# ZhangHaoyang493/News_Recsys

Hardware: AMD Instinct MI355X
Metric: impressions/sec at batch 65536 (embedding hot path forward) (higher is better)
Workload: dtype f32

## Files before the change

news_recsys_amd/csrc/nrx_interact.hip:

```cpp
#include "nrx_common.h"

namespace {

__global__ __launch_bounds__(NRX_BLOCK) void bag_pool_fwd_kernel(const float* __restrict__ emb, const float* __restrict__ mask,
                                                                 int64_t batch, int L, int D, float* __restrict__ out) {
    const int64_t total = batch * (int64_t)D;
    for (int64_t i = (int64_t)blockIdx.x * NRX_BLOCK + threadIdx.x; i < total; i += (int64_t)gridDim.x * NRX_BLOCK) {
        const int64_t b = i / D;
        const int d = (int)(i - b * D);
        const float* e = emb + (b * L) * (int64_t)D + d;
        float acc = 0.f, den = 0.f;
        if (mask != nullptr) {
            const float* m = mask + b * (int64_t)L;
            for (int l = 0; l < L; ++l) {
#pragma clang fp contract(off)
                const float w = m[l];
                den += w;
                acc += e[(int64_t)l * D] * w;
            }
            out[i] = acc / (den + 1e-8f);
        } else {
            for (int l = 0; l < L; ++l) acc += e[(int64_t)l * D];
            out[i] = acc / (float)L;
        }
    }
}

template <bool VEC>
__global__ __launch_bounds__(NRX_BLOCK) void bag_pool_bwd_kernel(const float* __restrict__ g_out, const float* __restrict__ mask,
                                                                 int64_t batch, int L, int D, float* __restrict__ g_emb) {
    const int lane = threadIdx.x & 63;
    const int64_t wave = (int64_t)blockIdx.x * (NRX_BLOCK / 64) + (threadIdx.x >> 6);
    const int64_t nwaves = (int64_t)gridDim.x * (NRX_BLOCK / 64);
    const int n = L * D;
    for (int64_t b = wave; b < batch; b += nwaves) {
        float den = (float)L;
        if (mask != nullptr) {
            float part = 0.f;
            for (int l = lane; l < L; l += NRX_WAVE) part += mask[b * (int64_t)L + l];
            den = nrx_wave_sum(part) + 1e-8f;
        }
        const float* gb = g_out + b * (int64_t)D;
        const float* mb = mask ? mask + b * (int64_t)L : nullptr;
        float* ob = g_emb + b * (int64_t)n;
        if (VEC) {
            const unsigned q = (unsigned)D >> 2;
            for (unsigned e4 = lane; e4 < (unsigned)n >> 2; e4 += NRX_WAVE) {
                const unsigned l = e4 / q, d = (e4 - l * q) * 4;
                const float4 g = *reinterpret_cast<const float4*>(gb + d);
                const float m = mb ? mb[l] : 1.0f;
                float4 o = make_float4(g.x / den, g.y / den, g.z / den, g.w / den);
                if (mb) o = make_float4(o.x * m, o.y * m, o.z * m, o.w * m);
                *reinterpret_cast<float4*>(ob + (size_t)e4 * 4) = o;
            }
        } else {
            for (int e = lane; e < n; e += NRX_WAVE) {
                const int l = e / D, d = e - l * D;
                const float g = gb[d] / den;
                ob[e] = mb ? g * mb[l] : g;
            }
        }
    }
}

__device__ __forceinline__ float4 ld4(const float* p, int k0, int D, bool vec) {
    float4 v;
    if (vec) {
        v = *reinterpret_cast<const float4*>(p);
    } else {
        v.x = p[0];
        v.y = (k0 + 1 < D) ? p[1] : 0.f;
        v.z = (k0 + 2 < D) ? p[2] : 0.f;
        v.w = (k0 + 3 < D) ? p[3] : 0.f;
    }
    return v;
}

template <int QLOG2>
__global__ __launch_bounds__(NRX_BLOCK) void fm_fwd_kernel(const float* __restrict__ feat, int64_t ld, int F, int D,
                                                           int64_t batch, float* __restrict__ fm_out, bool vec,
                                                           float* __restrict__ sums = nullptr, int64_t sums_ld = 0) {
    constexpr int Q = 1 << QLOG2;
    constexpr int TB = NRX_BLOCK / Q;
    const int q = threadIdx.x & (Q - 1);
    const int64_t b = (int64_t)blockIdx.x * TB + (threadIdx.x >> QLOG2);
    const bool live = b < batch;
    float total = 0.f;
    for (int kc = 0; kc < D; kc += 4 * Q) {
        const int k0 = kc + q * 4;
        float first = 0.f;
        float4 s = make_float4(0.f, 0.f, 0.f, 0.f), sq = s;
        if (live && k0 < D) {
            const float* row = feat + b * ld + k0;
            for (int f = 0; f < F; ++f) {
                float4 v = ld4(row + (int64_t)f * D, k0, D, vec);
                if (k0 == 0) { first += v.x; v.x = 0.f; }
                s.x += v.x; s.y += v.y; s.z += v.z; s.w += v.w;
                sq.x += v.x * v.x; sq.y += v.y * v.y; sq.z += v.z * v.z; sq.w += v.w * v.w;
            }
        }
        total += 0.5f * ((s.x * s.x - sq.x) + (s.y * s.y - sq.y) + (s.z * s.z - sq.z) + (s.w * s.w - sq.w)) + first;
        if (sums != nullptr && live && k0 < D) {
            float* dst = sums + b * sums_ld + k0;
            const float v0 = k0 == 0 ? first : s.x;
            dst[0] = v0;
            if (k0 + 1 < D) dst[1] = s.y;
            if (k0 + 2 < D) dst[2] = s.z;
            if (k0 + 3 < D) dst[3] = s.w;
        }
    }
#pragma unroll
    for (int off = Q / 2; off > 0; off >>= 1) total += __shfl_xor(total, off, 64);
    if (live && q == 0) fm_out[b] = total;
}

template <int QLOG2>
__global__ __launch_bounds__(NRX_BLOCK) void fm_bwd_kernel(const float* __restrict__ feat, int64_t ld, int F, int D, int64_t batch,
                                                           const float* __restrict__ g_fm, const float* g_in, int64_t g_in_ld,
                                                           float* g_feat, int64_t g_ld, bool vec) {
    constexpr int Q = 1 << QLOG2;
    constexpr int TB = NRX_BLOCK / Q;
    constexpr int U = 8;
    const int q = threadIdx.x & (Q - 1);
    const int64_t b = (int64_t)blockIdx.x * TB + (threadIdx.x >> QLOG2);
    if (b >= batch) return;
    const float gl = g_fm[b];
    const bool gvec = vec && (g_ld & 3) == 0 && ((reinterpret_cast<uintptr_t>(g_feat) & 15u) == 0) &&
                      (g_in == nullptr || ((g_in_ld & 3) == 0 && (reinterpret_cast<uintptr_t>(g_in) & 15u) == 0));
    for (int kc = 0; kc < D; kc += 4 * Q) {
        const int k0 = kc + q * 4;
        if (k0 >= D) continue;
        const float* row = feat + b * ld + k0;
        const float* irow = g_in ? g_in + b * g_in_ld + k0 : nullptr;
        float* grow = g_feat + b * g_ld + k0;
        float4 s = make_float4(0.f, 0.f, 0.f, 0.f);
        int f = 0;
        for (; f + U <= F; f += U) {
            float4 v[U];
#pragma unroll
            for (int u = 0; u < U; ++u) v[u] = ld4(row + (int64_t)(f + u) * D, k0, D, vec);
#pragma unroll
            for (int u = 0; u < U; ++u) { s.x += v[u].x; s.y += v[u].y; s.z += v[u].z; s.w += v[u].w; }
        }
        for (; f < F; ++f) {
            const float4 v = ld4(row + (int64_t)f * D, k0, D, vec);
            s.x += v.x; s.y += v.y; s.z += v.z; s.w += v.w;
        }
        f = 0;
        if (gvec && k0 + 4 <= D) {
            for (; f + U <= F; f += U) {
                float4 v[U], up[U];
#pragma unroll
                for (int u = 0; u < U; ++u) {
                    v[u] = ld4(row + (int64_t)(f + u) * D, k0, D, vec);
                    up[u] = irow ? *reinterpret_cast<const float4*>(irow + (int64_t)(f + u) * D) : make_float4(0.f, 0.f, 0.f, 0.f);
                }
#pragma unroll
                for (int u = 0; u < U; ++u) {
                    float4 g = make_float4(gl * (s.x - v[u].x), gl * (s.y - v[u].y), gl * (s.z - v[u].z), gl * (s.w - v[u].w));
                    if (k0 == 0) g.x = gl;
                    *reinterpret_cast<float4*>(grow + (int64_t)(f + u) * D) = make_float4(up[u].x + g.x, up[u].y + g.y, up[u].z + g.z, up[u].w + g.w);
                }
            }
        }
        for (; f < F; ++f) {
            const float4 v = ld4(row + (int64_t)f * D, k0, D, vec);
            float g[4] = {gl * (s.x - v.x), gl * (s.y - v.y), gl * (s.z - v.z), gl * (s.w - v.w)};
            if (k0 == 0) g[0] = gl;
            float* gp = grow + (int64_t)f * D;
            const float* ip = irow ? irow + (int64_t)f * D : nullptr;
#pragma unroll
            for (int j = 0; j < 4; ++j)
                if (k0 + j < D) gp[j] = (ip ? ip[j] : 0.f) + g[j];
        }
    }
}

template <int R, int V>
struct RowRegs {
    float v[R][V];
};

template <int R, int V>
__device__ __forceinline__ void row_load(RowRegs<R, V>& x, const float* p, int D, int lane) {
#pragma unroll
    for (int r = 0; r < R; ++r) {
        const int c = (r * 64 + lane) * V;
        if (V == 4) {
            float4 t = make_float4(0.f, 0.f, 0.f, 0.f);
            if (c < D) t = *reinterpret_cast<const float4*>(p + c);
            x.v[r][0] = t.x; x.v[r][1 % V] = t.y; x.v[r][2 % V] = t.z; x.v[r][3 % V] = t.w;
        } else {
            x.v[r][0] = (c < D) ? p[c] : 0.f;
        }
    }
}
// ... 526 lines not shown
            NRX_GLOBAL nrx_f32x4* o = (NRX_GLOBAL nrx_f32x4*)(a->out + b * a->out_ld);
#pragma unroll
            for (int u = EARLY ? N : 0; u < 2 * N; ++u) {
                const float4 v = u < N ? x0[u] : xl[u - N];
                nrx_f32x4 t;
                t.x = v.x; t.y = v.y; t.z = v.z; t.w = v.w;
                NRX_GLOBAL nrx_f32x4* dst = o + (u < N ? 0 : W / 4) + (u < N ? u : u - N) * Q + q;
                if (STNT) __builtin_nontemporal_store(t, dst);
                else *dst = t;
            }
        }
    }
}

int ceil_log2i(int x) {
    int l = 0;
    while ((1 << l) < x) ++l;
    return l;
}

unsigned stream_grid(int64_t items, int per_block) {
    int64_t g = (items + per_block - 1) / per_block;
    const int64_t cap = 256 * 8;
    if (g > cap) g = cap;
    if (g < 1) g = 1;
    return (unsigned)g;
}

#define NRX_QSWITCH(qlog2, ...)               \
    switch (qlog2) {                           \
        case 0: { constexpr int QL = 0; __VA_ARGS__; } break; \
        case 1: { constexpr int QL = 1; __VA_ARGS__; } break; \
        case 2: { constexpr int QL = 2; __VA_ARGS__; } break; \
        case 3: { constexpr int QL = 3; __VA_ARGS__; } break; \
        case 4: { constexpr int QL = 4; __VA_ARGS__; } break; \
        case 5: { constexpr int QL = 5; __VA_ARGS__; } break; \
        default: { constexpr int QL = 6; __VA_ARGS__; } break; \
    }

#define NRX_RSWITCH(R_, V_, ...)                                   \
    if (V_ == 4) {                                                  \
        constexpr int VV = 4;                                       \
        if (R_ <= 1) { constexpr int RR = 1; __VA_ARGS__; }                \
        else if (R_ <= 2) { constexpr int RR = 2; __VA_ARGS__; }           \
        else if (R_ <= 4) { constexpr int RR = 4; __VA_ARGS__; }           \
        else { constexpr int RR = 8; __VA_ARGS__; }                        \
    } else {                                                        \
        constexpr int VV = 1;                                       \
        if (R_ <= 1) { constexpr int RR = 1; __VA_ARGS__; }                \
        else if (R_ <= 2) { constexpr int RR = 2; __VA_ARGS__; }           \
        else if (R_ <= 4) { constexpr int RR = 4; __VA_ARGS__; }           \
        else if (R_ <= 8) { constexpr int RR = 8; __VA_ARGS__; }           \
        else if (R_ <= 16) { constexpr int RR = 16; __VA_ARGS__; }         \
        else { constexpr int RR = 32; __VA_ARGS__; }                       \
    }

}

extern "C" int nrx_bag_pool_fwd(const float* emb, const float* mask, int64_t batch, int32_t bag_len,
                                int32_t dim, float* out, void* stream) {
    NRX_TRACE();
    NRX_REQUIRE(emb && out && batch >= 0 && bag_len >= 1 && dim >= 1, "nrx_bag_pool_fwd: bad argument");
    if (batch == 0) return NRX_OK;
    hipLaunchKernelGGL(bag_pool_fwd_kernel, dim3(stream_grid(batch * dim, NRX_BLOCK)), dim3(NRX_BLOCK), 0,
                       reinterpret_cast<hipStream_t>(stream), emb, mask, batch, bag_len, dim, out);
    NRX_LAUNCH_CHECK("nrx_bag_pool_fwd");
    return NRX_OK;
}

extern "C" int nrx_bag_pool_bwd(const float* g_out, const float* mask, int64_t batch, int32_t bag_len,
                                int32_t dim, float* g_emb, void* stream) {
    NRX_TRACE();
    NRX_REQUIRE(g_out && g_emb && batch >= 0 && bag_len >= 1 && dim >= 1, "nrx_bag_pool_bwd: bad argument");
    if (batch == 0) return NRX_OK;
    const bool vec = (dim & 3) == 0 && nrx_aligned16(g_out) && nrx_aligned16(g_emb);
    if (vec) hipLaunchKernelGGL(bag_pool_bwd_kernel<true>, dim3(stream_grid(batch, NRX_BLOCK / 64)), dim3(NRX_BLOCK), 0,
                                reinterpret_cast<hipStream_t>(stream), g_out, mask, batch, bag_len, dim, g_emb);
    else hipLaunchKernelGGL(bag_pool_bwd_kernel<false>, dim3(stream_grid(batch, NRX_BLOCK / 64)), dim3(NRX_BLOCK), 0,
                            reinterpret_cast<hipStream_t>(stream), g_out, mask, batch, bag_len, dim, g_emb);
    NRX_LAUNCH_CHECK("nrx_bag_pool_bwd");
    return NRX_OK;
}

extern "C" int nrx_fm_fwd(const float* feat, int64_t ld, int32_t n_fields, int32_t dim, int64_t batch,
                          float* fm_out, void* stream) {
    NRX_TRACE();
    NRX_REQUIRE(feat && fm_out && n_fields >= 1 && dim >= 1 && batch >= 0 && ld >= (int64_t)n_fields * dim,
                "nrx_fm_fwd: bad argument");
    if (batch == 0) return NRX_OK;
    int ql = ceil_log2i((dim + 3) / 4);
    if (ql > 6) ql = 6;
    const bool vec = (dim & 3) == 0 && (ld & 3) == 0 && nrx_aligned16(feat);
    const int tb = NRX_BLOCK >> ql;
    const unsigned grid = (unsigned)((batch + tb - 1) / tb);
    NRX_QSWITCH(ql, { hipLaunchKernelGGL((fm_fwd_kernel<QL>), dim3(grid), dim3(NRX_BLOCK), 0, reinterpret_cast<hipStream_t>(stream),
                                         feat, ld, n_fields, dim, batch, fm_out, vec); });
    NRX_LAUNCH_CHECK("nrx_fm_fwd");
    return NRX_OK;
}

extern "C" int nrx_fm_fwd_train(const float* feat, int64_t ld, int32_t n_fields, int32_t dim, int64_t batch,
                                float* fm_out, float* fm_sums, int64_t sums_ld, void* stream) {
    NRX_TRACE();
    NRX_REQUIRE(feat && fm_out && fm_sums && n_fields >= 1 && dim >= 1 && batch >= 0 && ld >= (int64_t)n_fields * dim && sums_ld >= dim,
                "nrx_fm_fwd_train: bad argument");
    if (batch == 0) return NRX_OK;
    int ql = ceil_log2i((dim + 3) / 4);
    if (ql > 6) ql = 6;
    const bool vec = (dim & 3) == 0 && (ld & 3) == 0 && nrx_aligned16(feat);
    const int tb = NRX_BLOCK >> ql;
    const unsigned grid = (unsigned)((batch + tb - 1) / tb);
    NRX_QSWITCH(ql, { hipLaunchKernelGGL((fm_fwd_kernel<QL>), dim3(grid), dim3(NRX_BLOCK), 0, reinterpret_cast<hipStream_t>(stream),
                                         feat, ld, n_fields, dim, batch, fm_out, vec, fm_sums, sums_ld); });
    NRX_LAUNCH_CHECK("nrx_fm_fwd_train");
    return NRX_OK;
}

extern "C" int nrx_fm_bwd(const float* feat, int64_t ld, int32_t n_fields, int32_t dim, int64_t batch,
                          const float* g_fm, const float* g_in, int64_t g_in_ld, float* g_feat, int64_t g_ld, void* stream) {
    NRX_TRACE();
    NRX_REQUIRE(feat && g_fm && g_feat && n_fields >= 1 && dim >= 1 && batch >= 0, "nrx_fm_bwd: bad argument");
    if (batch == 0) return NRX_OK;
    int ql = ceil_log2i((dim + 3) / 4);
    if (ql > 6) ql = 6;
    const bool vec = (dim & 3) == 0 && (ld & 3) == 0 && nrx_aligned16(feat);
    const int tb = NRX_BLOCK >> ql;
    const unsigned grid = (unsigned)((batch + tb - 1) / tb);
    NRX_QSWITCH(ql, { hipLaunchKernelGGL((fm_bwd_kernel<QL>), dim3(grid), dim3(NRX_BLOCK), 0, reinterpret_cast<hipStream_t>(stream),
                                         feat, ld, n_fields, dim, batch, g_fm, g_in, g_in_ld, g_feat, g_ld, vec); });
    NRX_LAUNCH_CHECK("nrx_fm_bwd");
    return NRX_OK;
}

namespace {
constexpr int FH_BLOCKS = 64;
__global__ __launch_bounds__(NRX_BLOCK) void fm_head_fwd_kernel(const float* __restrict__ logit, const float* __restrict__ bias, float* __restrict__ out,
                                                                int64_t batch) {
    const float b = bias != nullptr ? bias[0] : 0.f;
    for (int64_t i = (int64_t)blockIdx.x * NRX_BLOCK + threadIdx.x; i < batch; i += (int64_t)gridDim.x * NRX_BLOCK) {
        const float x = b + logit[i];
        out[i] = 1.0f / (1.0f + expf(-x));
    }
}
__global__ __launch_bounds__(NRX_BLOCK) void fm_head_bwd_kernel(const float* __restrict__ g_out, int64_t g_stride, const float* __restrict__ out,
                                                                float* __restrict__ g_logit, float* __restrict__ g_bias, uint32_t* __restrict__ state,
                                                                int64_t batch) {
    __shared__ float s_w[NRX_BLOCK / 64];
    __shared__ uint32_t s_last;
    const int64_t chunk = (batch + gridDim.x - 1) / gridDim.x;
    const int64_t lo = (int64_t)blockIdx.x * chunk, hi = lo + chunk < batch ? lo + chunk : batch;
    float acc = 0.f;
    for (int64_t i = lo + threadIdx.x; i < hi; i += NRX_BLOCK) {
        const float p = out[i];
        const float g = g_out[i * g_stride] * (p * (1.0f - p));
        g_logit[i] = g;
        acc += g;
    }
    if (g_bias == nullptr) return;
    acc = nrx_wave_sum(acc);
    if ((threadIdx.x & 63) == 0) s_w[threadIdx.x >> 6] = acc;
    __syncthreads();
    float* partial = reinterpret_cast<float*>(state + 8);
    if (threadIdx.x == 0) {
        partial[blockIdx.x] = (s_w[0] + s_w[1]) + (s_w[2] + s_w[3]);
        __threadfence();
        s_last = atomicAdd(&state[0], 1u) == gridDim.x - 1 ? 1u : 0u;
    }
    __syncthreads();
    if (s_last && threadIdx.x < 64) {
        __threadfence();
        float v = (int)threadIdx.x < (int)gridDim.x ? __hip_atomic_load(&partial[threadIdx.x], __ATOMIC_RELAXED, __HIP_MEMORY_SCOPE_AGENT) : 0.f;
        v = nrx_wave_sum(v);
        if (threadIdx.x == 0) {
            g_bias[0] = v;
            state[0] = 0;
        }
    }
}
}

extern "C" int nrx_fm_head_fwd(const float* logit, const float* bias, float* out, int64_t batch, void* stream) {
    NRX_TRACE();
    NRX_REQUIRE(logit && out && batch >= 0, "nrx_fm_head_fwd: bad argument");
    if (batch == 0) return NRX_OK;
    const int64_t g = (batch + NRX_BLOCK - 1) / NRX_BLOCK;
    hipLaunchKernelGGL(fm_head_fwd_kernel, dim3((unsigned)(g < 1024 ? g : 1024)), dim3(NRX_BLOCK), 0, reinterpret_cast<hipStream_t>(stream), logit, bias, out, batch);
    NRX_LAUNCH_CHECK("nrx_fm_head_fwd");
    return NRX_OK;
}

extern "C" int64_t nrx_fm_head_state_bytes(void) { return 32 + FH_BLOCKS * 4; }

// ... 326 lines not shown
```

news_recsys_amd/csrc/nrx_route_feat.hip:

```cpp
#include <cstring>

#include "nrx_common.h"

namespace {

constexpr int RF_THREADS = 256;
#ifndef NRX_RF_ROUNDS
#define NRX_RF_ROUNDS 16
#endif
constexpr int RF_ROUNDS = NRX_RF_ROUNDS;
constexpr int RF_TILE = RF_THREADS * RF_ROUNDS;
constexpr int RF_WAVES = RF_THREADS / 64;
constexpr int RF_MAX_WORLD = 64;

struct RouteFeatArgs {
    const void* ids[NRX_MAX_FEATURES];
    int64_t batch;
    int64_t capf;
    int32_t n_feats, world, idx64, tiles;
    int32_t* send_ids;
    int32_t* send_pos;
    int32_t* slot;
    int64_t* counts;
    int64_t* overflow;
// ... 379 lines not shown
    if (last_of_feat) {
        tiles_before_in_group(a->tile0[f], s_feat);
        groups_before(a->tile0[f], s_feat);
    }
#endif
    __syncthreads();
    const int64_t cap = a->cap, B = a->batch;
    const int L = a->bag_len[f];
    const uint64_t magic_l = a->magic_len[f];
    const int32_t tag0 = (int32_t)(f * B);
    const int64_t ntag_r = (int64_t)n * B;
#pragma unroll
    for (int j = 0; j < RF_ROUNDS; ++j) {
        if (owner[j] < 0) continue;
        const int o = owner[j];
        const int64_t i = i0 + j * RF_THREADS + tid;
        const int pt = RUNS ? rank[j] : s_cell[j * RF_WAVES + wid][o] + rank[j];
        const int64_t k = (int64_t)s_base[o] + pt;
        const int32_t smp = RUNS ? (int32_t)smp0 + local_sample(j) : (L == 1 ? (int32_t)i : (int32_t)__umul64hi((uint64_t)i, magic_l));
#ifdef NRX_RB_NO_STORE
        if (k < 0) {
#else
        if (k < cap) {
#endif
            const int64_t d = (int64_t)o * cap + k;
            a->send_rows[d] = val[j];
            if (!RUNS) a->send_tag[d] = tag0 + smp;
            a->send_w[d] = wt[j];
        }
        if (RUNS && ((opn | cls) >> j) & 1u) {
            int32_t* r = a->send_run + ((int64_t)o * ntag_r + tag0 + smp) * 2;
            if ((opn >> j) & 1u) r[0] = (int32_t)(k < cap ? k : cap);
            if ((cls >> j) & 1u) r[1] = (int32_t)(k + 1 < cap ? k + 1 : cap);
        }
    }
    if (last_of_feat && tid < W) a->counts2d[(int64_t)tid * n + f] = (int64_t)s_base[tid] + s_tot[tid] - s_feat[tid];
    if (w == T - 1 && tid == 0) {
        long long worst = 0;
        for (int o = 0; o < W; ++o) {
            const long long c = (long long)s_base[o] + s_tot[o];
            worst = c > worst ? c : worst;
        }
        atomicMax(reinterpret_cast<long long*>(a->overflow), worst);
    }
    __syncthreads();
    if (w == T - 1 && tid == 0) {
        __hip_atomic_store(&a->ctl[2], mark, __ATOMIC_RELAXED, __HIP_MEMORY_SCOPE_AGENT);
        __hip_atomic_store(&a->ctl[0], 0u, __ATOMIC_RELAXED, __HIP_MEMORY_SCOPE_AGENT);
    }
}

__global__ __launch_bounds__(NRX_BLOCK) void inbox_transpose_kernel(const int32_t* __restrict__ a_in, int32_t* __restrict__ a_out,
                                                                   const int32_t* __restrict__ b_in, int32_t* __restrict__ b_out, int world, int n,
                                                                   int64_t capf) {
    const int64_t total = (int64_t)world * n * capf;
    for (int64_t i = ((int64_t)blockIdx.x * NRX_BLOCK + threadIdx.x) * 4; i < total; i += (int64_t)gridDim.x * NRX_BLOCK * 4) {
        const int64_t run = i / capf, k = i - run * capf;
        const int s = (int)(run / n), f = (int)(run - (int64_t)s * n);
        const int64_t o = ((int64_t)f * world + s) * capf + k;
        typedef int nrx_i32x4t __attribute__((ext_vector_type(4)));
        *reinterpret_cast<nrx_i32x4t*>(a_out + o) = *reinterpret_cast<const nrx_i32x4t*>(a_in + i);
        if (b_in != nullptr) *reinterpret_cast<nrx_i32x4t*>(b_out + o) = *reinterpret_cast<const nrx_i32x4t*>(b_in + i);
    }
}

#ifndef NRX_GP_R
#define NRX_GP_R 8
#endif
constexpr int GP_R = NRX_GP_R;
struct GatherPlaceArgs {
    const float* table[NRX_MAX_FEATURES];
    int64_t rows[NRX_MAX_FEATURES];
    int32_t col[NRX_MAX_FEATURES];
    float* peer[RF_MAX_WORLD];
    const int32_t* oid;
    const int32_t* opos;
    int64_t bp, capf, ld, out_rows;
    int32_t n, world;
    int32_t* status;
};
static_assert(sizeof(GatherPlaceArgs) <= 3584, "kernarg budget");

typedef unsigned nrx_gp_u32x2 __attribute__((ext_vector_type(2)));
template <int QLOG2, typename TS = float>
__global__ __launch_bounds__(NRX_BLOCK) void gather_place_feat_kernel(const GatherPlaceArgs args_in_kernarg) {
    const NRX_CONST GatherPlaceArgs* a = nrx_kernarg<GatherPlaceArgs>();
    constexpr int Q = 1 << QLOG2, TB = NRX_BLOCK / Q;
    const int q = threadIdx.x & (Q - 1);
    const int64_t bp = a->bp;
    const int n = a->n;
    for (int64_t b = (int64_t)blockIdx.x * TB + (threadIdx.x >> QLOG2); b < bp; b += (int64_t)gridDim.x * TB) {
        const int s = (int)(b / a->capf);
        float* __restrict__ out = a->peer[s];
        auto fetch = [&](int f0, int32_t* id, int32_t* pos) {
#pragma unroll
            for (int r = 0; r < GP_R; ++r) {
                const int f = f0 + r < n ? f0 + r : n - 1;
                id[r] = nrx_gconst<int32_t>(a->oid)[(int64_t)f * bp + b];
                pos[r] = nrx_gconst<int32_t>(a->opos)[(int64_t)f * bp + b];
            }
        };
        auto process = [&](int f0, const int32_t* id, int32_t* pos) {
            float4 v[GP_R];
            [[maybe_unused]] nrx_gp_u32x2 raw[GP_R];
            [[maybe_unused]] bool use[GP_R];
#pragma unroll
            for (int r = 0; r < GP_R; ++r) {
                const int f = f0 + r < n ? f0 + r : n - 1;
                v[r] = make_float4(0.f, 0.f, 0.f, 0.f);
                if constexpr (sizeof(TS) == 2) {
                    const uint64_t tb = reinterpret_cast<uint64_t>(a->table[f]);
                    const uint32_t tb_lo = __builtin_amdgcn_readfirstlane((uint32_t)tb), tb_hi = __builtin_amdgcn_readfirstlane((uint32_t)(tb >> 32));
                    const uint32_t nr = __builtin_amdgcn_readfirstlane((uint32_t)(a->rows[f] > 0x7fffffff ? 0x7fffffff : a->rows[f]));
                    const NRX_GLOBAL nrx_gp_u32x2* base = (const NRX_GLOBAL nrx_gp_u32x2*)(((uint64_t)tb_hi << 32) | tb_lo);
                    use[r] = f0 + r < n && pos[r] >= 0 && id[r] > 0 && (uint32_t)id[r] < nr;
                    raw[r] = __builtin_nontemporal_load(base + ((int64_t)(use[r] ? id[r] : 0) * Q + q));
                }
                if (f0 + r >= n || pos[r] < 0) { pos[r] = -1; continue; }
                if (id[r] < 0 || (int64_t)id[r] >= a->rows[f]) {
                    if (q == 0) nrx_report_oob(a->status, f, b, id[r]);
                    continue;
                }
                if constexpr (sizeof(TS) != 2) {
                    if (id[r] != 0) v[r] = nrx_ldg4_nt(a->table[f], (int64_t)id[r] * Q + q);
                }
            }
#pragma unroll
            for (int r = 0; r < GP_R; ++r) {
                if (pos[r] < 0) continue;
                const int f = f0 + r;
                if ((int64_t)pos[r] >= a->out_rows) {
                    if (q == 0) nrx_report_oob(a->status, f, b, pos[r]);
                    continue;
                }
                if constexpr (sizeof(TS) == 2) {
                    if (use[r]) v[r] = nrx_bf16x4_to_f32(raw[r].x, raw[r].y);
                }
                nrx_stg4(out, ((int64_t)pos[r] * a->ld + a->col[f]) / 4 + q, v[r]);
            }
        };
        int32_t ida[GP_R], posa[GP_R], idb[GP_R], posb[GP_R];
        fetch(0, ida, posa);
        for (int f0 = 0; f0 < n; f0 += 2 * GP_R) {
            if (f0 + GP_R < n) fetch(f0 + GP_R, idb, posb);
            process(f0, ida, posa);
            if (f0 + GP_R >= n) break;
            if (f0 + 2 * GP_R < n) fetch(f0 + 2 * GP_R, ida, posa);
            process(f0 + GP_R, idb, posb);
        }
    }
}

__global__ __launch_bounds__(NRX_BLOCK) void shard_dest_combine_kernel(const int32_t* __restrict__ slot, const int32_t* __restrict__ dest_req, int n, int64_t batch,
                                                                      int64_t capf, int64_t recv_row0, int rank, int shift, int32_t* __restrict__ out) {
    const int f = blockIdx.y;
    const uint32_t un = (uint32_t)n, ucapf = (uint32_t)capf;
    for (int64_t b = (int64_t)blockIdx.x * NRX_BLOCK + threadIdx.x; b < batch; b += (int64_t)gridDim.x * NRX_BLOCK) {
        const int64_t p = (int64_t)f * batch + b;
        const int32_t sl = slot[p];
        int32_t r = -1;
        if (sl >= 0) {
            const uint32_t ok = (uint32_t)sl / un, o = ok / ucapf, k = ok - o * ucapf;
            const int32_t d = dest_req[((int64_t)o * n + f) * capf + k];
            const int64_t row = d >= 0 ? (int64_t)d : recv_row0 + ((int64_t)rank * capf + k) * n + f;
            r = (int32_t)(((int64_t)o << shift) | row);
        }
        out[p] = r;
    }
}

bool all_resident(const void* kernel, int64_t blocks) {
    static thread_local const void* cached_k[4] = {nullptr, nullptr, nullptr, nullptr};
    static thread_local int64_t cached_cap[4] = {0, 0, 0, 0};
    int64_t capacity = -1;
    for (int i = 0; i < 4; ++i)
        if (cached_k[i] == kernel) capacity = cached_cap[i];
    if (capacity < 0) {
        int per_cu = 0, dev = 0, cus = 0;
        if (hipOccupancyMaxActiveBlocksPerMultiprocessor(&per_cu, kernel, RF_THREADS, 0) != hipSuccess || hipGetDevice(&dev) != hipSuccess ||
            hipDeviceGetAttribute(&cus, hipDeviceAttributeMultiprocessorCount, dev) != hipSuccess)
            return false;
        capacity = (int64_t)per_cu * cus;
        for (int i = 0; i < 4; ++i)
            if (cached_k[i] == nullptr) { cached_k[i] = kernel; cached_cap[i] = capacity; break; }
    }
    return blocks <= capacity;
}

}

extern "C" int nrx_shard_dest_combine(const int32_t* slot, const int32_t* dest_req, int32_t n_feats, int64_t batch, int64_t capf, int64_t recv_row0,
                                      int32_t rank, int32_t world, int32_t shift, int32_t* dest_out, void* stream) {
    NRX_TRACE();
    NRX_REQUIRE(slot && dest_req && dest_out && n_feats >= 1 && batch >= 0 && capf >= 1 && rank >= 0 && rank < world, "nrx_shard_dest_combine: bad argument");
    NRX_REQUIRE(shift >= 1 && shift <= 30 && (int64_t)world <= (1ll << (31 - shift)) && recv_row0 + (int64_t)world * capf * n_feats <= (1ll << shift),
                "nrx_shard_dest_combine: (owner << shift) | row must fit 31 bits");
    if (batch == 0) return NRX_OK;
    NRX_REQUIRE(capf < 0x7fffffffLL && n_feats <= NRX_MAX_FEATURES, "nrx_shard_dest_combine: capf must fit 31 bits, n_feats <= %d", NRX_MAX_FEATURES);
    int64_t blocks = (batch + NRX_BLOCK - 1) / NRX_BLOCK;
    if (blocks > 1024) blocks = 1024;
    hipLaunchKernelGGL(shard_dest_combine_kernel, dim3((unsigned)blocks, (unsigned)n_feats), dim3(NRX_BLOCK), 0, reinterpret_cast<hipStream_t>(stream), slot, dest_req, (int)n_feats,
                       batch, capf, recv_row0, (int)rank, (int)shift, dest_out);
    NRX_LAUNCH_CHECK("nrx_shard_dest_combine");
    return NRX_OK;
}

namespace {
template <typename TS>
int gather_place_feat_launch(const char* who, const void* const* tables, const int64_t* table_rows, const int32_t* feat_col, int32_t n_feats, int32_t world,
                                     int64_t capf, const int32_t* owner_ids, const int32_t* owner_pos, int32_t dim, float* const* peer_out,
                                     int64_t out_ld, int64_t out_rows, int32_t* status, void* stream) {
    NRX_REQUIRE(tables && table_rows && feat_col && owner_ids && owner_pos && peer_out, "%s: null argument", who);
    NRX_REQUIRE(n_feats >= 1 && n_feats <= NRX_MAX_FEATURES && world >= 1 && world <= RF_MAX_WORLD && capf >= 1, "%s: bad sizes", who);
    if (!(dim == 16 || dim == 32 || dim == 64 || dim == 128 || dim == 256) || (out_ld & 3) != 0) {
        nrx_set_error("%s: dim must be 16 / 32 / 64 / 128 / 256 and out_ld a multiple of 4", who);
        return NRX_ERR_UNSUPPORTED;
    }
    GatherPlaceArgs a;
    memset(&a, 0, sizeof(a));
    for (int i = 0; i < n_feats; ++i) {
        NRX_REQUIRE(tables[i] != nullptr && (reinterpret_cast<uintptr_t>(tables[i]) & (sizeof(TS) == 2 ? 7u : 15u)) == 0 && (feat_col[i] & 3) == 0,
                    "%s: feature %d: aligned table and column", who, i);
        NRX_REQUIRE(sizeof(TS) != 2 || table_rows[i] >= 1, "%s: feature %d: a bf16 arena has at least its dummy row", who, i);
        a.table[i] = reinterpret_cast<const float*>(tables[i]);
        a.rows[i] = table_rows[i];
        a.col[i] = feat_col[i];
    }
    for (int s = 0; s < world; ++s) {
        NRX_REQUIRE(peer_out[s] != nullptr && nrx_aligned16(peer_out[s]), "%s: peer %d: null / unaligned buffer", who, s);
        a.peer[s] = peer_out[s];
    }
    a.oid = owner_ids;
    a.opos = owner_pos;
    a.bp = (int64_t)world * capf;
    a.capf = capf;
    a.ld = out_ld;
    a.out_rows = out_rows;
    a.n = n_feats;
    a.world = world;
    a.status = status;
    const int ql = dim == 16 ? 2 : dim == 32 ? 3 : dim == 64 ? 4 : dim == 128 ? 5 : 6;
    const int64_t tb = NRX_BLOCK >> ql;
    int64_t blocks = (a.bp + tb - 1) / tb;
    if (blocks > 8192) blocks = 8192;
    hipStream_t st = reinterpret_cast<hipStream_t>(stream);
    if (ql == 2) hipLaunchKernelGGL((gather_place_feat_kernel<2, TS>), dim3((unsigned)blocks), dim3(NRX_BLOCK), 0, st, a);
    else if (ql == 3) hipLaunchKernelGGL((gather_place_feat_kernel<3, TS>), dim3((unsigned)blocks), dim3(NRX_BLOCK), 0, st, a);
    else if (ql == 4) hipLaunchKernelGGL((gather_place_feat_kernel<4, TS>), dim3((unsigned)blocks), dim3(NRX_BLOCK), 0, st, a);
    else if (ql == 5) hipLaunchKernelGGL((gather_place_feat_kernel<5, TS>), dim3((unsigned)blocks), dim3(NRX_BLOCK), 0, st, a);
    else hipLaunchKernelGGL((gather_place_feat_kernel<6, TS>), dim3((unsigned)blocks), dim3(NRX_BLOCK), 0, st, a);
    NRX_LAUNCH_CHECK(who);
    return NRX_OK;
}
}

extern "C" int nrx_gather_place_feat(const float* const* tables, const int64_t* table_rows, const int32_t* feat_col, int32_t n_feats, int32_t world,
                                     int64_t capf, const int32_t* owner_ids, const int32_t* owner_pos, int32_t dim, float* const* peer_out,
                                     int64_t out_ld, int64_t out_rows, int32_t* status, void* stream) {
    NRX_TRACE();
    return gather_place_feat_launch<float>("nrx_gather_place_feat", reinterpret_cast<const void* const*>(tables), table_rows, feat_col, n_feats, world, capf,
                                           owner_ids, owner_pos, dim, peer_out, out_ld, out_rows, status, stream);
}

extern "C" int nrx_gather_place_feat_bf16(const uint16_t* const* tables, const int64_t* table_rows, const int32_t* feat_col, int32_t n_feats, int32_t world,
                                          int64_t capf, const int32_t* owner_ids, const int32_t* owner_pos, int32_t dim, float* const* peer_out,
                                          int64_t out_ld, int64_t out_rows, int32_t* status, void* stream) {
    NRX_TRACE();
    return gather_place_feat_launch<uint16_t>("nrx_gather_place_feat_bf16", reinterpret_cast<const void* const*>(tables), table_rows, feat_col, n_feats, world,
                                              capf, owner_ids, owner_pos, dim, peer_out, out_ld, out_rows, status, stream);
}

extern "C" int64_t nrx_route_feat_state_bytes(int32_t n_feats, int64_t batch, int32_t world) {
    if (n_feats < 1 || n_feats > NRX_MAX_FEATURES || batch < 0 || world < 1 || world > RF_MAX_WORLD) return -1;
    const int64_t tiles = (batch + RF_TILE - 1) / RF_TILE;
    return 512 + (int64_t)n_feats * (tiles > 0 ? tiles : 1) * world * 8;
}

extern "C" int nrx_route_feat(const void* const* ids, int32_t n_feats, int64_t batch, int32_t index_bits, int32_t world, int64_t capf,
                              int32_t* send_ids, int32_t* send_pos, int32_t* slot, int64_t* counts, int64_t* overflow, void* state, void* stream) {
    NRX_TRACE();
    NRX_REQUIRE(ids != nullptr && n_feats >= 1 && n_feats <= NRX_MAX_FEATURES, "nrx_route_feat: n_feats must be in [1, %d]", NRX_MAX_FEATURES);
    NRX_REQUIRE(world >= 1 && world <= RF_MAX_WORLD, "nrx_route_feat: world must be in [1, %d]", RF_MAX_WORLD);
    NRX_REQUIRE(index_bits == 32 || index_bits == 64, "nrx_route_feat: index_bits must be 32 or 64");
    NRX_REQUIRE(batch >= 0 && batch < 0x7fffffffLL && capf >= 1, "nrx_route_feat: bad batch / capf");
    NRX_REQUIRE((int64_t)world * capf * n_feats < 0x7fffffffLL, "nrx_route_feat: world * capf * n_feats must stay below 2^31 (slot is int32)");
    NRX_REQUIRE(send_ids && slot && counts && overflow && state, "nrx_route_feat: null buffer");
    if (batch == 0) return NRX_OK;
    RouteFeatArgs a;
    memset(&a, 0, sizeof(a));
    for (int i = 0; i < n_feats; ++i) {
        NRX_REQUIRE(ids[i] != nullptr, "nrx_route_feat: feature %d: null ids", i);
        a.ids[i] = ids[i];
    }
    a.batch = batch;
    a.capf = capf;
    a.n_feats = n_feats;
    a.world = world;
    a.idx64 = index_bits == 64;
    a.tiles = (int32_t)((batch + RF_TILE - 1) / RF_TILE);
    a.send_ids = send_ids;
    a.send_pos = send_pos;
    a.slot = slot;
    a.counts = counts;
    a.overflow = overflow;
    a.ctl = reinterpret_cast<uint32_t*>(state);
    a.agg = reinterpret_cast<unsigned long long*>(reinterpret_cast<char*>(state) + 512);
    a.use_ticket = world > 1 && !all_resident(reinterpret_cast<const void*>(route_feat_kernel), (int64_t)n_feats * a.tiles);
    hipLaunchKernelGGL(route_feat_kernel, dim3((unsigned)(n_feats * a.tiles)), dim3(RF_THREADS), 0, reinterpret_cast<hipStream_t>(stream), a);
    NRX_LAUNCH_CHECK("nrx_route_feat");
    return NRX_OK;
}

extern "C" int64_t nrx_route_bags_one_state_bytes(const int32_t* bag_lens, int32_t n_feats, int64_t batch, int32_t world) {
    if (bag_lens == nullptr || n_feats < 1 || n_feats > NRX_MAX_FEATURES || batch < 0 || world < 1 || world > RF_MAX_WORLD) return -1;
    int64_t tiles = 0;
    for (int f = 0; f < n_feats; ++f) tiles += (batch * bag_lens[f] + RF_TILE - 1) / RF_TILE;
    return 64 + ((tiles > 0 ? tiles : 1) + tiles / RB_GROUP + 1) * world * 8;
}

extern "C" int nrx_route_bags_one(const void* const* ids, const float* const* weights, const int32_t* bag_lens, int32_t n_feats, int32_t index_bits,
                                  int64_t batch, int32_t world, int64_t cap, int32_t* send_rows, int32_t* send_tag, float* send_w, int64_t* counts2d,
                                  int64_t* overflow, void* state, void* stream) {
    NRX_TRACE();
    NRX_REQUIRE(ids && bag_lens && n_feats >= 1 && n_feats <= NRX_MAX_FEATURES, "nrx_route_bags_one: n_feats must be in [1, %d]", NRX_MAX_FEATURES);
    NRX_REQUIRE(index_bits == 32 || index_bits == 64, "nrx_route_bags_one: index_bits must be 32 or 64");
    NRX_REQUIRE(world >= 1 && world <= RF_MAX_WORLD && cap >= 1 && cap * world <= 0x7fffffffLL && batch >= 0, "nrx_route_bags_one: bad world / cap / batch");
    NRX_REQUIRE((int64_t)n_feats * batch <= 0x7fffffffLL, "nrx_route_bags_one: n_feats * batch must fit 31 bits");
    NRX_REQUIRE(send_rows && send_tag && send_w && counts2d && overflow && state, "nrx_route_bags_one: null buffer");
    RouteBagsArgs a;
    memset(&a, 0, sizeof(a));
    int64_t tiles = 0, total = 0;
    for (int f = 0; f < n_feats; ++f) {
        NRX_REQUIRE(bag_lens[f] >= 1 && (batch == 0 || ids[f] != nullptr), "nrx_route_bags_one: feature %d: bad ids / bag_len", f);
// ... 117 lines not shown
```

Measured before the change: 1.106 billion.

## Add paired-field FM forward kernel for dim 16 and LDS-staged gather-place

Adds an FM forward kernel specialised for dim 16 in which two lanes groups load alternating fields and exchange them via DPP, so each row is read as full cache lines with more loads in flight. Rewrites the gather-place kernel to first stage owner ids and positions for the whole block tile in LDS, doing bounds checks in a coalesced pass, then software-pipelines table loads across features. The intent is to cut scattered index loads and raise memory-level parallelism on the embedding hot path. It adds dynamic shared memory proportional to feature count, extra syncs, and an environment-controlled fallback.

```diff
diff --git a/news_recsys_amd/csrc/nrx_interact.hip b/news_recsys_amd/csrc/nrx_interact.hip
--- a/news_recsys_amd/csrc/nrx_interact.hip
+++ b/news_recsys_amd/csrc/nrx_interact.hip
@@ -1,4 +1,6 @@
 #include "nrx_common.h"
+#include <cstdlib>
+#include <cstring>
 
 namespace {
 
@@ -112,6 +114,78 @@
 #pragma unroll
     for (int off = Q / 2; off > 0; off >>= 1) total += __shfl_xor(total, off, 64);
     if (live && q == 0) fm_out[b] = total;
+}
+
+__device__ __forceinline__ float fm_close_q4(const float4& s, const float4& sq, float first) {
+#pragma clang fp contract(off)
+    const float tx = __builtin_fmaf(s.x, s.x, -sq.x), ty = __builtin_fmaf(s.y, s.y, -sq.y);
+    const float mz = s.z * s.z, mw = s.w * s.w;
+    const float tz = mz - sq.z, tw = mw - sq.w;
+    return __builtin_fmaf(0.5f, ((tx + ty) + tz) + tw, first);
+}
+
+template <int U, bool TRAIN>
+__global__ __launch_bounds__(NRX_BLOCK) void fm_fwd_lines_kernel(const float* __restrict__ feat, int64_t ld, int F, int64_t batch,
+                                                                 float* __restrict__ fm_out, float* __restrict__ sums, int64_t sums_ld) {
+    constexpr int Q = 4, D = 16;
+    constexpr int TB = NRX_BLOCK / (2 * Q);
+    const int q = threadIdx.x & (Q - 1);
+    const int par = (threadIdx.x >> 2) & 1;
+    const int64_t b = (int64_t)blockIdx.x * TB + (threadIdx.x >> 3);
+    const bool live = b < batch;
+    const int k0 = q * 4;
+    const int np = (F + 1) >> 1;
+    const float* row = feat + (live ? b : batch - 1) * ld + k0;
+    float total = 0.f;
+    float first = 0.f;
+    float4 s = make_float4(0.f, 0.f, 0.f, 0.f), sq = s;
+    auto add = [&](float4 v) {
+        if (k0 == 0) { first += v.x; v.x = 0.f; }
+        s.x += v.x; s.y += v.y; s.z += v.z; s.w += v.w;
+        sq.x = __builtin_fmaf(v.x, v.x, sq.x); sq.y = __builtin_fmaf(v.y, v.y, sq.y);
+        sq.z = __builtin_fmaf(v.z, v.z, sq.z); sq.w = __builtin_fmaf(v.w, v.w, sq.w);
+    };
+    auto partner = [](const float4& v) {
+        return make_float4(nrx_dpp<0x104>(v.x), nrx_dpp<0x104>(v.y), nrx_dpp<0x104>(v.z), nrx_dpp<0x104>(v.w));
+    };
+    for (int j0 = 0; j0 < np; j0 += U) {
+        float4 v[U];
+#pragma unroll
+        for (int u = 0; u < U; ++u) {
+            const int j = j0 + u < np ? j0 + u : np - 1;
+            const int f = 2 * j + par < F ? 2 * j + par : F - 1;
+            v[u] = nrx_ldg4(row + f * D, 0);
+        }
+        __builtin_amdgcn_sched_barrier(0);
+        if (j0 + U <= np) {
+#pragma unroll
+            for (int u = 0; u < U; ++u) {
+                const float4 w = partner(v[u]);
+                add(v[u]);
+                if (u + 1 < U || 2 * (j0 + u) + 1 < F) add(w);
+            }
+        } else {
+#pragma unroll
+            for (int u = 0; u < U; ++u) {
+                if (j0 + u < np) {
+                    const float4 w = partner(v[u]);
+                    add(v[u]);
+                    if (2 * (j0 + u) + 1 < F) add(w);
+                }
+            }
+        }
+    }
+    total += fm_close_q4(s, sq, first);
+    if (TRAIN && live && par == 0) {
+        float* dst = sums + b * sums_ld + k0;
+        dst[0] = k0 == 0 ? first : s.x;
+        dst[1] = s.y;
+        dst[2] = s.z;
+        dst[3] = s.w;
+    }
+#pragma unroll
+    for (int off = Q / 2; off > 0; off >>= 1) total += __shfl_xor(total, off, 64);
+    if (live && (threadIdx.x & 7) == 0) fm_out[b] = total;
 }
 
 template <int QLOG2>
@@ -804,6 +878,27 @@
     return NRX_OK;
 }
 
+static bool fm_fwd_lines_ok(const float* feat, int64_t ld, int32_t dim) {
+    bool lines = dim == 16 && (ld & 31) == 0 && (reinterpret_cast<uintptr_t>(feat) & 127u) == 0;
+    if (const char* e = getenv("NRX_FM_FWD_FORM")) lines = lines && strcmp(e, "rows") != 0;
+    if (const char* e = getenv("NRX_FM_FWD_LOG"))
+        if (atoi(e) != 0) { fprintf(stderr, "nrx_fm_fwd: form=%s\n", lines ? "lines" : "rows"); fflush(stderr); }
+    return lines;
+}
+
+template <bool TRAIN>
+static void fm_fwd_lines_launch(const float* feat, int64_t ld, int32_t n_fields, int64_t batch, float* fm_out, float* sums, int64_t sums_ld,
+                                hipStream_t st) {
+    const int np = (n_fields + 1) / 2;
+    const unsigned grid = (unsigned)((batch + NRX_BLOCK / 8 - 1) / (NRX_BLOCK / 8));
+#define NRX_FM_LINES(UU) hipLaunchKernelGGL((fm_fwd_lines_kernel<UU, TRAIN>), dim3(grid), dim3(NRX_BLOCK), 0, st, feat, ld, n_fields, batch, fm_out, sums, sums_ld)
+    if (np <= 2) NRX_FM_LINES(2);
+    else if (np <= 4) NRX_FM_LINES(4);
+    else if (np <= 8) NRX_FM_LINES(8);
+    else NRX_FM_LINES(13);
+#undef NRX_FM_LINES
+}
+
 extern "C" int nrx_fm_fwd(const float* feat, int64_t ld, int32_t n_fields, int32_t dim, int64_t batch,
                           float* fm_out, void* stream) {
     NRX_TRACE();
@@ -813,6 +908,11 @@
     int ql = ceil_log2i((dim + 3) / 4);
     if (ql > 6) ql = 6;
     const bool vec = (dim & 3) == 0 && (ld & 3) == 0 && nrx_aligned16(feat);
+    if (fm_fwd_lines_ok(feat, ld, dim)) {
+        fm_fwd_lines_launch<false>(feat, ld, n_fields, batch, fm_out, nullptr, 0, reinterpret_cast<hipStream_t>(stream));
+        NRX_LAUNCH_CHECK("nrx_fm_fwd");
+        return NRX_OK;
+    }
     const int tb = NRX_BLOCK >> ql;
     const unsigned grid = (unsigned)((batch + tb - 1) / tb);
     NRX_QSWITCH(ql, { hipLaunchKernelGGL((fm_fwd_kernel<QL>), dim3(grid), dim3(NRX_BLOCK), 0, reinterpret_cast<hipStream_t>(stream),
@@ -830,6 +930,11 @@
     int ql = ceil_log2i((dim + 3) / 4);
     if (ql > 6) ql = 6;
     const bool vec = (dim & 3) == 0 && (ld & 3) == 0 && nrx_aligned16(feat);
+    if (fm_fwd_lines_ok(feat, ld, dim)) {
+        fm_fwd_lines_launch<true>(feat, ld, n_fields, batch, fm_out, fm_sums, sums_ld, reinterpret_cast<hipStream_t>(stream));
+        NRX_LAUNCH_CHECK("nrx_fm_fwd_train");
+        return NRX_OK;
+    }
     const int tb = NRX_BLOCK >> ql;
     const unsigned grid = (unsigned)((batch + tb - 1) / tb);
     NRX_QSWITCH(ql, { hipLaunchKernelGGL((fm_fwd_kernel<QL>), dim3(grid), dim3(NRX_BLOCK), 0, reinterpret_cast<hipStream_t>(stream),
diff --git a/news_recsys_amd/csrc/nrx_route_feat.hip b/news_recsys_amd/csrc/nrx_route_feat.hip
--- a/news_recsys_amd/csrc/nrx_route_feat.hip
+++ b/news_recsys_amd/csrc/nrx_route_feat.hip
@@ -485,72 +485,121 @@
 static_assert(sizeof(GatherPlaceArgs) <= 3584, "kernarg budget");
 
 typedef unsigned nrx_gp_u32x2 __attribute__((ext_vector_type(2)));
+typedef int nrx_gp_i32x2 __attribute__((ext_vector_type(2)));
+template <typename TS>
+struct GpRaw { typedef nrx_f32x4 type; };
+template <>
+struct GpRaw<uint16_t> { typedef nrx_gp_u32x2 type; };
+
 template <int QLOG2, typename TS = float>
 __global__ __launch_bounds__(NRX_BLOCK) void gather_place_feat_kernel(const GatherPlaceArgs args_in_kernarg) {
     const NRX_CONST GatherPlaceArgs* a = nrx_kernarg<GatherPlaceArgs>();
-    constexpr int Q = 1 << QLOG2, TB = NRX_BLOCK / Q;
-    const int q = threadIdx.x & (Q - 1);
+    constexpr int Q = 1 << QLOG2, TB = NRX_BLOCK / Q, R = GP_R;
+    typedef typename GpRaw<TS>::type raw_t;
+    extern __shared__ __attribute__((aligned(16))) nrx_gp_i32x2 s_ent[];
+    const int tid = threadIdx.x;
+    const int q = tid & (Q - 1), sb = tid >> QLOG2;
     const int64_t bp = a->bp;
     const int n = a->n;
-    for (int64_t b = (int64_t)blockIdx.x * TB + (threadIdx.x >> QLOG2); b < bp; b += (int64_t)gridDim.x * TB) {
-        const int s = (int)(b / a->capf);
-        float* __restrict__ out = a->peer[s];
-        auto fetch = [&](int f0, int32_t* id, int32_t* pos) {
-#pragma unroll
-            for (int r = 0; r < GP_R; ++r) {
-                const int f = f0 + r < n ? f0 + r : n - 1;
-                id[r] = nrx_gconst<int32_t>(a->oid)[(int64_t)f * bp + b];
-                pos[r] = nrx_gconst<int32_t>(a->opos)[(int64_t)f * bp + b];
-            }
-        };
-        auto process = [&](int f0, const int32_t* id, int32_t* pos) {
-            float4 v[GP_R];
-            [[maybe_unused]] nrx_gp_u32x2 raw[GP_R];
-            [[maybe_unused]] bool use[GP_R];
-#pragma unroll
-            for (int r = 0; r < GP_R; ++r) {
-                const int f = f0 + r < n ? f0 + r : n - 1;
-                v[r] = make_float4(0.f, 0.f, 0.f, 0.f);
-                if constexpr (sizeof(TS) == 2) {
-                    const uint64_t tb = reinterpret_cast<uint64_t>(a->table[f]);
-                    const uint32_t tb_lo = __builtin_amdgcn_readfirstlane((uint32_t)tb), tb_hi = __builtin_amdgcn_readfirstlane((uint32_t)(tb >> 32));
-                    const uint32_t nr = __builtin_amdgcn_readfirstlane((uint32_t)(a->rows[f] > 0x7fffffff ? 0x7fffffff : a->rows[f]));
-                    const NRX_GLOBAL nrx_gp_u32x2* base = (const NRX_GLOBAL nrx_gp_u32x2*)(((uint64_t)tb_hi << 32) | tb_lo);
-                    use[r] = f0 + r < n && pos[r] >= 0 && id[r] > 0 && (uint32_t)id[r] < nr;
-                    raw[r] = __builtin_nontemporal_load(base + ((int64_t)(use[r] ? id[r] : 0) * Q + q));
+    const int total = n * TB;
+    for (int64_t b0 = (int64_t)blockIdx.x * TB; b0 < bp; b0 += (int64_t)gridDim.x * TB) {
+        constexpr int PASS = 4;
+        for (int i0 = tid; i0 < total; i0 += PASS * NRX_BLOCK) {
+            int32_t id[PASS], pos[PASS];
+            int64_t nr[PASS];
+#pragma unroll
+            for (int u = 0; u < PASS; ++u) {
+                const int i = i0 + u * NRX_BLOCK < total ? i0 + u * NRX_BLOCK : total - 1;
+                const int f = i / TB;
+                const int64_t b = b0 + (i - f * TB);
+                const int64_t at = (int64_t)f * bp + (b < bp ? b : bp - 1);
+                id[u] = nrx_gconst<int32_t>(a->oid)[at];
+                pos[u] = nrx_gconst<int32_t>(a->opos)[at];
+                nr[u] = a->rows[f];
+            }
+#pragma unroll
+            for (int u = 0; u < PASS; ++u) {
+                const int i = i0 + u * NRX_BLOCK;
+                if (i >= total) break;
+                const int f = i / TB;
+                const int64_t b = b0 + (i - f * TB);
+                int32_t row = id[u], p = b < bp ? pos[u] : -1;
+                if (p >= 0) {
+                    if (row < 0 || (int64_t)row >= nr[u]) {
+                        nrx_report_oob(a->status, f, b, row);
+                        row = 0;
+                    }
+                    if ((int64_t)p >= a->out_rows) {
+                        nrx_report_oob(a->status, f, b, p);
+                        p = -1;
+                    }
                 }
-                if (f0 + r >= n || pos[r] < 0) { pos[r] = -1; continue; }
-                if (id[r] < 0 || (int64_t)id[r] >= a->rows[f]) {
-                    if (q == 0) nrx_report_oob(a->status, f, b, id[r]);
-                    continue;
+                nrx_gp_i32x2 e;
+                e.x = p >= 0 ? row : 0;
+                e.y = p;
+                s_ent[i] = e;
+            }
+        }
+        __syncthreads();
+        {
+            const int64_t b = b0 + sb < bp ? b0 + sb : bp - 1;
+            float* __restrict__ out = a->peer[(int)(b / a->capf)];
+            const nrx_gp_i32x2* s_my = s_ent + sb;
+            auto load = [&](int fv, int32_t row) -> raw_t {
+                const int f = __builtin_amdgcn_readfirstlane(fv);
+                return __builtin_nontemporal_load((const NRX_GLOBAL raw_t*)(a->table[f]) + (((int64_t)row << QLOG2) + q));
+            };
+            auto place = [&](int fv, nrx_gp_i32x2 e, const raw_t& r) {
+                const int f = __builtin_amdgcn_readfirstlane(fv);
+                if (e.y >= 0) {
+                    float4 v = make_float4(0.f, 0.f, 0.f, 0.f);
+                    if (e.x != 0) {
+                        if constexpr (sizeof(TS) == 2) v = nrx_bf16x4_to_f32(r.x, r.y);
+                        else v = make_float4(r.x, r.y, r.z, r.w);
+                    }
+                    nrx_stg4(out, ((int64_t)e.y * a->ld + a->col[f]) / 4 + q, v);
                 }
-                if constexpr (sizeof(TS) != 2) {
-                    if (id[r] != 0) v[r] = nrx_ldg4_nt(a->table[f], (int64_t)id[r] * Q + q);
+            };
+            nrx_gp_i32x2 e[R];
+            raw_t v[R];
+#pragma unroll
+            for (int u = 0; u < R; ++u) e[u] = s_my[(u < n ? u : n - 1) * TB];
+#pragma unroll
+            for (int u = 0; u < R; ++u)
+                if (u < n) v[u] = load(u, e[u].x);
+            int f0 = 0;
+            for (; f0 + 2 * R <= n; f0 += R) {
+                nrx_gp_i32x2 en[R];
+#pragma unroll
+                for (int u = 0; u < R; ++u) en[u] = s_my[(f0 + R + u) * TB];
+#pragma unroll
+                for (int u = 0; u < R; ++u) {
+                    place(f0 + u, e[u], v[u]);
+                    e[u] = en[u];
+                    v[u] = load(f0 + R + u, e[u].x);
                 }
             }
-#pragma unroll
-            for (int r = 0; r < GP_R; ++r) {
-                if (pos[r] < 0) continue;
-                const int f = f0 + r;
-                if ((int64_t)pos[r] >= a->out_rows) {
-                    if (q == 0) nrx_report_oob(a->status, f, b, pos[r]);
-                    continue;
+            {
+                nrx_gp_i32x2 en[R];
+#pragma unroll
+                for (int u = 0; u < R; ++u) {
+                    const int f = f0 + R + u;
+                    en[u] = s_my[(f < n ? f : n - 1) * TB];
                 }
-                if constexpr (sizeof(TS) == 2) {
-                    if (use[r]) v[r] = nrx_bf16x4_to_f32(raw[r].x, raw[r].y);
+#pragma unroll
+                for (int u = 0; u < R; ++u) {
+                    if (f0 + u < n) place(f0 + u, e[u], v[u]);
+                    if (f0 + R + u < n) {
+                        e[u] = en[u];
+                        v[u] = load(f0 + R + u, e[u].x);
+                    }
                 }
-                nrx_stg4(out, ((int64_t)pos[r] * a->ld + a->col[f]) / 4 + q, v[r]);
-            }
-        };
-        int32_t ida[GP_R], posa[GP_R], idb[GP_R], posb[GP_R];
-        fetch(0, ida, posa);
-        for (int f0 = 0; f0 < n; f0 += 2 * GP_R) {
-            if (f0 + GP_R < n) fetch(f0 + GP_R, idb, posb);
-            process(f0, ida, posa);
-            if (f0 + GP_R >= n) break;
-            if (f0 + 2 * GP_R < n) fetch(f0 + 2 * GP_R, ida, posa);
-            process(f0 + GP_R, idb, posb);
-        }
+#pragma unroll
+                for (int u = 0; u < R; ++u)
+                    if (f0 + R + u < n) place(f0 + R + u, e[u], v[u]);
+            }
+        }
+        __syncthreads();
     }
 }
 
@@ -624,7 +673,7 @@
     for (int i = 0; i < n_feats; ++i) {
         NRX_REQUIRE(tables[i] != nullptr && (reinterpret_cast<uintptr_t>(tables[i]) & (sizeof(TS) == 2 ? 7u : 15u)) == 0 && (feat_col[i] & 3) == 0,
                     "%s: feature %d: aligned table and column", who, i);
-        NRX_REQUIRE(sizeof(TS) != 2 || table_rows[i] >= 1, "%s: feature %d: a bf16 arena has at least its dummy row", who, i);
+        NRX_REQUIRE(table_rows[i] >= 1, "%s: feature %d: an arena has at least its dummy row", who, i);
         a.table[i] = reinterpret_cast<const float*>(tables[i]);
         a.rows[i] = table_rows[i];
         a.col[i] = feat_col[i];
@@ -646,12 +695,13 @@
     const int64_t tb = NRX_BLOCK >> ql;
     int64_t blocks = (a.bp + tb - 1) / tb;
     if (blocks > 8192) blocks = 8192;
+    const size_t lds = (size_t)n_feats * tb * 8;
     hipStream_t st = reinterpret_cast<hipStream_t>(stream);
-    if (ql == 2) hipLaunchKernelGGL((gather_place_feat_kernel<2, TS>), dim3((unsigned)blocks), dim3(NRX_BLOCK), 0, st, a);
-    else if (ql == 3) hipLaunchKernelGGL((gather_place_feat_kernel<3, TS>), dim3((unsigned)blocks), dim3(NRX_BLOCK), 0, st, a);
-    else if (ql == 4) hipLaunchKernelGGL((gather_place_feat_kernel<4, TS>), dim3((unsigned)blocks), dim3(NRX_BLOCK), 0, st, a);
-    else if (ql == 5) hipLaunchKernelGGL((gather_place_feat_kernel<5, TS>), dim3((unsigned)blocks), dim3(NRX_BLOCK), 0, st, a);
-    else hipLaunchKernelGGL((gather_place_feat_kernel<6, TS>), dim3((unsigned)blocks), dim3(NRX_BLOCK), 0, st, a);
+    if (ql == 2) hipLaunchKernelGGL((gather_place_feat_kernel<2, TS>), dim3((unsigned)blocks), dim3(NRX_BLOCK), lds, st, a);
+    else if (ql == 3) hipLaunchKernelGGL((gather_place_feat_kernel<3, TS>), dim3((unsigned)blocks), dim3(NRX_BLOCK), lds, st, a);
+    else if (ql == 4) hipLaunchKernelGGL((gather_place_feat_kernel<4, TS>), dim3((unsigned)blocks), dim3(NRX_BLOCK), lds, st, a);
+    else if (ql == 5) hipLaunchKernelGGL((gather_place_feat_kernel<5, TS>), dim3((unsigned)blocks), dim3(NRX_BLOCK), lds, st, a);
+    else hipLaunchKernelGGL((gather_place_feat_kernel<6, TS>), dim3((unsigned)blocks), dim3(NRX_BLOCK), lds, st, a);
     NRX_LAUNCH_CHECK(who);
     return NRX_OK;
 }
```

New measurement: 1.092 billion. 1.2% lower.
